# avianphysics/avian

Measured on NVIDIA H100. Metric: physics steps/sec on 100k-cube stack (broad phase + solver stage per step), higher is better.
Workload: dtype f32

## Files before the change

avian_b200/csrc/solver_dev.cuh:

```cuda
#pragma once
#include <cuda_pipeline.h>

#include "../../include/avian_b200.h"
#include "avn_math.cuh"

namespace avn {

enum { CP_N = 0, CP_T1 = 1, CP_TV = 2, CP_IDX = 3, CP_PT0 = 4, CP_PLANES = CP_PT0 + 3 * AVN_MAX_MANIFOLD_POINTS };
#define CP_ROW(k, r) (CP_PT0 + 3 * (k) + (r))
enum { CI_NP_MASK = 0x7, CI_ZERO1 = 1 << 4, CI_ZERO2 = 1 << 5, CI_NONDYN = 1 << 6, CI_TANGENT = 1 << 7,
       CI_VER1 = 1 << 8, CI_VER2 = 1 << 9 };
enum { BF_LOCK_MASK = 0x3f, BF_HAS_SOLVER_BODY = 1 << 8, BF_KINEMATIC = 1 << 9, BF_GYRO = 1 << 10, BF_DYNAMIC = 1 << 11,
       BF_CUSTOM_VEL = 1 << 12, BF_CUSTOM_POS = 1 << 13, BF_DOMINANCE_SHIFT = 16 };

enum { JP_IDX = 0,
       JP_R1 = 1,
       JP_R2 = 2,
       JP_CD = 3,
       JP_RD = 4,
       JP_A1 = 5,
       JP_A2 = 6,
       JP_B1 = 7,
       JP_B2 = 8,
       JP_LP = 9,
// ... 245 lines not shown
        case WV_WARM: return base + 1u + r;
        case WV_SOLVE: return base + 1u + unsigned(1 + it) * k + r;
        case WV_IP: return base + 1u + unsigned(1 + iters) * k;
        default: return base + 2u + unsigned(1 + iters) * k + r;
    }
}
__device__ __forceinline__ unsigned ld_acquire(const unsigned* p) {
    unsigned v;
    asm volatile("ld.acquire.gpu.global.u32 %0, [%1];" : "=r"(v) : "l"(p) : "memory");
    return v;
}
__device__ __forceinline__ void st_relaxed(unsigned* p, unsigned v) { asm volatile("st.relaxed.gpu.global.u32 [%0], %1;" ::"l"(p), "r"(v) : "memory"); }
__device__ __forceinline__ void fence_acq_rel() { asm volatile("fence.acq_rel.gpu;" ::: "memory"); }
__device__ __forceinline__ Vec4<float> ld4_cg(const Vec4<float>* p) {
    float4 v = __ldcg(reinterpret_cast<const float4*>(p));
    return mk4<float>(v.x, v.y, v.z, v.w);
}
__device__ __forceinline__ Vec4<double> ld4_cg(const Vec4<double>* p) {
    double2 a = __ldcg(reinterpret_cast<const double2*>(p)), b = __ldcg(reinterpret_cast<const double2*>(p) + 1);
    return mk4<double>(a.x, a.y, b.x, b.y);
}
template <bool WAVE, class S> __device__ __forceinline__ Vec4<S> ldm(const Vec4<S>* p) { return WAVE ? ld4_cg(p) : ld4(p); }
template <bool WAVE, class S> __device__ __forceinline__ Vec4<S> pc_load(const Vec4<S>* p) { return ldm<WAVE>(p); }

template <bool EXACT = true>
__device__ __forceinline__ void wave_wait(const unsigned* ver, bool need1, int b1, unsigned e1, bool need2, int b2, unsigned e2, int* watchdog,
                                          unsigned* seen1 = nullptr, unsigned* seen2 = nullptr) {
    for (unsigned spins = 0;; ++spins) {
        if (need1) { const unsigned v = ld_acquire(ver + b1); need1 = EXACT ? v != e1 : v < e1; if (seen1) *seen1 = v; }
        if (need2) { const unsigned v = ld_acquire(ver + b2); need2 = EXACT ? v != e2 : v < e2; if (seen2) *seen2 = v; }
        if (__all_sync(0xffffffffu, !(need1 || need2))) break;
        if (spins > (1u << 22)) { *watchdog = 1; break; }
    }
}
__device__ __forceinline__ void wave_publish(unsigned* ver, bool need1, int b1, unsigned e1, bool need2, int b2, unsigned e2) {
    fence_acq_rel();
    if (need1) st_relaxed(ver + b1, e1 + 1u);
    if (need2) st_relaxed(ver + b2, e2 + 1u);
}

constexpr int STAGE_ROWS = 3 * AVN_MAX_MANIFOLD_POINTS;
template <class S> __device__ __forceinline__ Vec4<S>* stage_base() {
    extern __shared__ __align__(32) unsigned char avn_stage_raw[];
    return reinterpret_cast<Vec4<S>*>(avn_stage_raw);
}
__device__ __forceinline__ void stage_copy(Vec4<float>* dst, const Vec4<float>* src) { __pipeline_memcpy_async(dst, src, 16); }
__device__ __forceinline__ void stage_copy(Vec4<double>* dst, const Vec4<double>* src) {
    __pipeline_memcpy_async(dst, src, 16);
    __pipeline_memcpy_async(reinterpret_cast<char*>(dst) + 16, reinterpret_cast<const char*>(src) + 16, 16);
}
template <class S> __host__ __device__ constexpr size_t stage_bytes(int threads, int max_points = AVN_MAX_MANIFOLD_POINTS) {
    return size_t(4 * max_points) * threads * sizeof(Vec4<S>);
}

template <class S, int PASS, int MAXP = AVN_MAX_MANIFOLD_POINTS>
__device__ __forceinline__ void contact_item(const DevSolver<S>& d, int slot) {
    const size_t MP = size_t(d.Mpad);
    Vec4<S>* c = d.cst + slot;
    Vec4<S> hidx = ld4(&c[CP_IDX * MP]);
    const int info = as_int(hidx.z);
    const int np = info & CI_NP_MASK;
    if (np == 0) return;
    const int b1 = as_int(hidx.x), b2 = as_int(hidx.y);
    Vec4<S> hn = mk4<S>(0, 0, 0, 0), ht1 = hn, htv = hn;
    BodyInertia<S> in1 = zero_inertia<S>(), in2 = zero_inertia<S>();
    Vec4<S> PC[MAXP];
    constexpr bool SOLVE = (PASS == PASS_SOLVE_BIAS || PASS == PASS_RELAX);
    Vec4<S>* const stage = stage_base<S>() + threadIdx.x;
    const int T = blockDim.x;
#define ROW_A(k) stage[(3 * (k) + 0) * T]
#define ROW_B(k) stage[(3 * (k) + 1) * T]
#define ROW_D(k) stage[(3 * (k) + 2) * T]
    {
        hn = ld4(&c[CP_N * MP]);
        ht1 = ld4(&c[CP_T1 * MP]);
        if (SOLVE) htv = ld4(&c[CP_TV * MP]);
        if (!(info & CI_ZERO1)) in1 = unpack_inertia(ld4(&d.inr[2 * b1]), ld4(&d.inr[2 * b1 + 1]));
        if (!(info & CI_ZERO2)) in2 = unpack_inertia(ld4(&d.inr[2 * b2]), ld4(&d.inr[2 * b2 + 1]));
#pragma unroll
        for (int k = 0; k < MAXP; ++k) {
            if (k < np) {
                stage_copy(&ROW_A(k), &c[size_t(CP_ROW(k, 0)) * MP]);
                stage_copy(&ROW_B(k), &c[size_t(CP_ROW(k, 1)) * MP]);
                if (PASS == PASS_RESTITUTION || (SOLVE && (info & CI_TANGENT))) stage_copy(&ROW_D(k), &c[size_t(CP_ROW(k, 2)) * MP]);
            }
        }
    }
    __pipeline_commit();
    Vec4<S> l1 = ld4(&d.vel[2 * b1]), a1 = ld4(&d.vel[2 * b1 + 1]);
    Vec4<S> l2 = ld4(&d.vel[2 * b2]), a2 = ld4(&d.vel[2 * b2 + 1]);
    Vec4<S> dp1, dq1, dp2, dq2;
    if (SOLVE) {
        dp1 = ld4(&d.dlt[2 * b1]); dq1 = ld4(&d.dlt[2 * b1 + 1]);
        dp2 = ld4(&d.dlt[2 * b2]); dq2 = ld4(&d.dlt[2 * b2 + 1]);
    }
#pragma unroll
    for (int k = 0; k < MAXP; ++k)
        if (k < np) PC[k] = pc_load<false>(pc_ptr(d, k, slot));
    __pipeline_wait_prior(0);
    V3<S> v1 = xyz(l1), w1 = xyz(a1), v2 = xyz(l2), w2 = xyz(a2);
    const V3<S> n = xyz(hn), t1 = xyz(ht1);
    const V3<S> t2 = cross(t1, n);

    if (PASS == PASS_WARM) {
#pragma unroll
        for (int k = 0; k < MAXP; ++k) {
// ... 63 lines not shown
                            nx = limit * (nx / l);
                            ny = limit * (ny / l);
                        }
                        S dx = nx - PC[k].z, dy = ny - PC[k].w;
                        PC[k].z = nx;
                        PC[k].w = ny;
                        imp = dx * t1 + dy * t2;
                    }
                    apply_impulse(v1, w1, v2, w2, in1, in2, r1, r2, imp);
                }
            }
        }
    } else {
        const S e = ht1.w;
        if (e == S(0)) return;
        const int iterations = np > 1 ? d.rest_iters : 1;
        for (int it = 0; it < iterations; ++it) {
#pragma unroll
            for (int k = 0; k < MAXP; ++k) {
                if (k < np) {
                    const Vec4<S> PAk = ROW_A(k), PBk = ROW_B(k), PDk = ROW_D(k);
                    if (PDk.w > -d.rest_threshold || PC[k].y == S(0)) continue;
                    V3<S> r1 = xyz(PAk), r2 = xyz(PBk);
                    V3<S> relv = (v2 + cross(w2, r2)) - (v1 + cross(w1, r1));
                    S vn = dot(relv, n);
                    S impulse = -PBk.w * (vn + e * PDk.w);
                    S new_impulse = avn_max(PC[k].x + impulse, S(0));
                    impulse = new_impulse - PC[k].x;
                    PC[k].x = new_impulse;
                    PC[k].y = PC[k].y + impulse;
                    apply_impulse(v1, w1, v2, w2, in1, in2, r1, r2, impulse * n);
                }
            }
        }
    }
    if (PASS != PASS_WARM) {
#pragma unroll
        for (int k = 0; k < MAXP; ++k)
            if (k < np) pc_store(pc_ptr(d, k, slot), PC[k]);
    }
    if (!(info & CI_ZERO1)) {
        st4(&d.vel[2 * b1], mk4<S>(v1.x, v1.y, v1.z, S(0)));
        st4(&d.vel[2 * b1 + 1], mk4<S>(w1.x, w1.y, w1.z, S(0)));
    }
    if (!(info & CI_ZERO2)) {
        st4(&d.vel[2 * b2], mk4<S>(v2.x, v2.y, v2.z, S(0)));
        st4(&d.vel[2 * b2 + 1], mk4<S>(w2.x, w2.y, w2.z, S(0)));
    }
#undef ROW_A
#undef ROW_B
#undef ROW_D
}

template <class S, int PASS, int MAXP>
__device__ __forceinline__ void wave_contact_item(const DevSolver<S>& d, int slot, int s, int it, bool relax) {
    constexpr bool SOLVE = PASS == PASS_SOLVE_BIAS;
    relax = SOLVE && relax;
    const size_t MP = size_t(d.Mpad);
    const Vec4<S>* c = d.cst + slot;
    const Vec4<S> hidx = ld4(&c[CP_IDX * MP]);
    const int info = as_int(hidx.z);
    const int np = info & CI_NP_MASK;
    const int b1 = as_int(hidx.x), b2 = as_int(hidx.y);
    Vec4<S>* const stage = stage_base<S>() + threadIdx.x;
    const int T = blockDim.x;
#define ROW_A(k) stage[(3 * (k) + 0) * T]
#define ROW_B(k) stage[(3 * (k) + 1) * T]
#define ROW_D(k) stage[(3 * (k) + 2) * T]
#define ROW_PC(k) stage[(3 * MAXP + (k)) * T]
    Vec4<S> hn = mk4<S>(0, 0, 0, 0), ht1 = hn, htv = hn;
    BodyInertia<S> in1 = zero_inertia<S>(), in2 = zero_inertia<S>();
    if (np != 0) {
        hn = ld4(&c[CP_N * MP]);
        ht1 = ld4(&c[CP_T1 * MP]);
        if (SOLVE) htv = ld4(&c[CP_TV * MP]);
        if (!(info & CI_ZERO1)) in1 = unpack_inertia(ld4(&d.inr[2 * b1]), ld4(&d.inr[2 * b1 + 1]));
        if (!(info & CI_ZERO2)) in2 = unpack_inertia(ld4(&d.inr[2 * b2]), ld4(&d.inr[2 * b2 + 1]));
#pragma unroll 1
        for (int k = 0; k < np; ++k) {
            stage_copy(&ROW_A(k), &c[size_t(CP_ROW(k, 0)) * MP]);
            stage_copy(&ROW_B(k), &c[size_t(CP_ROW(k, 1)) * MP]);
            if (SOLVE && (info & CI_TANGENT)) stage_copy(&ROW_D(k), &c[size_t(CP_ROW(k, 2)) * MP]);
        }
    }
    __pipeline_commit();
    const bool ver1 = np != 0 && (info & CI_VER1), ver2 = np != 0 && (info & CI_VER2);
    const int rk = as_int(hidx.w);
    const int k1 = (rk >> 8) & 0xff, k2 = (rk >> 24) & 0xff;
    const int kind = SOLVE ? (relax ? WV_RELAX : WV_SOLVE) : WV_WARM;
    const unsigned e1 = wave_event(kind, it, s, d.iters, k1, rk & 0xff);
    const unsigned e2 = wave_event(kind, it, s, d.iters, k2, (rk >> 16) & 0xff);
    int* const watchdog = d.any_restitution + FLAG_WAVE;
    const V3<S> n = xyz(hn), t1 = xyz(ht1);
    const Soft<S> soft = (info & CI_NONDYN) ? d.soft_nondyn : d.soft_dyn;
    unsigned biased_points = 0;
    unsigned seen1 = 0u, seen2 = 0u;

    if (SOLVE) {
        AVN_TRACE_T(t_d0);
        const int sd = relax ? s : s - 1;
        if (sd >= 0)
            wave_wait<false>(d.ver, ver1, b1, wave_event(WV_IP, 0, sd, d.iters, k1, 0) + 1u, ver2, b2, wave_event(WV_IP, 0, sd, d.iters, k2, 0) + 1u,
                             watchdog, &seen1, &seen2);
        __pipeline_wait_prior(0);
        if (np != 0) {
            const Vec4<S> dp1 = ld4_cg(&d.dlt[2 * b1]), dq1 = ld4_cg(&d.dlt[2 * b1 + 1]);
            const Vec4<S> dp2 = ld4_cg(&d.dlt[2 * b2]), dq2 = ld4_cg(&d.dlt[2 * b2 + 1]);
            Q4<S> q1; q1.x = dq1.x; q1.y = dq1.y; q1.z = dq1.z; q1.w = dq1.w;
            Q4<S> q2; q2.x = dq2.x; q2.y = dq2.y; q2.z = dq2.z; q2.w = dq2.w;
            const V3<S> delta_translation = xyz(dp2) - xyz(dp1);
#pragma unroll
            for (int k = 0; k < MAXP; ++k) {
                if (k >= np) break;
                const Vec4<S> PAk = ROW_A(k), PBk = ROW_B(k);
                V3<S> rr1 = qrot(q1, xyz(PAk)), rr2 = qrot(q2, xyz(PBk));
                V3<S> dsep = delta_translation + (rr2 - rr1);
                const S separation = dot(dsep, n) + PAk.w;
                const S meff = PBk.w;
                const bool separated = separation > S(0), biased = !separated && !relax;
                ROW_A(k).w = separated ? separation / d.h : biased ? avn_max(soft.bias * separation, -d.max_overlap_speed) : S(-0.0);
                ROW_B(k).w = biased ? soft.mass_scale * meff : meff;
                biased_points |= unsigned(biased) << k;
            }
        }
#ifdef AVN_WAVE_TRACE
        if (np != 0 && ROW_A(0).w == S(1.2345e33)) d.any_restitution[1] = 2;
        AVN_TRACE_ADD(d, 5, clock64() - t_d0);
#endif
    }

    AVN_TRACE_T(t_w0);
    wave_wait(d.ver, ver1 && seen1 != e1, b1, e1, ver2 && seen2 != e2, b2, e2, watchdog);
    AVN_TRACE_ADD(d, 0, clock64() - t_w0);
    if (np == 0) return;
    AVN_TRACE_T(t_l0);
    const Vec4<S> l1 = ld4_cg(&d.vel[2 * b1]), a1 = ld4_cg(&d.vel[2 * b1 + 1]);
    const Vec4<S> l2 = ld4_cg(&d.vel[2 * b2]), a2 = ld4_cg(&d.vel[2 * b2 + 1]);
    {
        Vec4<S> pc[MAXP];
#pragma unroll
        for (int k = 0; k < MAXP; ++k)
            if (k < np) pc[k] = pc_load<true>(pc_ptr(d, k, slot));
#pragma unroll
        for (int k = 0; k < MAXP; ++k)
            if (k < np) ROW_PC(k) = pc[k];
    }
    if (!SOLVE) __pipeline_wait_prior(0);
#ifdef AVN_WAVE_TRACE
    if ((l1.x + a1.x + l2.x + a2.x) == S(1.2345e33)) d.any_restitution[1] = 2;
    AVN_TRACE_T(t_c0);
    AVN_TRACE_ADD(d, 1, t_c0 - t_l0);
#endif
    V3<S> v1 = xyz(l1), w1 = xyz(a1), v2 = xyz(l2), w2 = xyz(a2);
    const V3<S> t2 = cross(t1, n);

    if (!SOLVE) {
#pragma unroll 1
        for (int k = 0; k < np; ++k) {
            const Vec4<S> PAk = ROW_A(k), PBk = ROW_B(k), pck = ROW_PC(k);
            V3<S> r1 = xyz(PAk), r2 = xyz(PBk);
            S tx = (info & CI_TANGENT) ? pck.z : S(0), ty = (info & CI_TANGENT) ? pck.w : S(0);
            V3<S> p = d.warm_coeff * ((pck.x * n + tx * t1) + ty * t2);
            apply_impulse(v1, w1, v2, w2, in1, in2, r1, r2, p);
        }
    } else {
        const bool tangent = (info & CI_TANGENT) != 0;
#pragma unroll 1
        for (int k = 0; k < np; ++k) {
            const Vec4<S> PAk = ROW_A(k), PBk = ROW_B(k);
            Vec4<S> pck = ROW_PC(k);
            V3<S> r1 = xyz(PAk), r2 = xyz(PBk);
            V3<S> relv = (v2 + cross(w2, r2)) - (v1 + cross(w1, r1));
            S vn = dot(relv, n);
            S acc = pck.x;
            const S C = ((biased_points >> k) & 1u) ? soft.impulse_scale * acc : S(0);
            S impulse = -PBk.w * (vn + PAk.w) - C;
            S new_impulse = avn_max(acc + impulse, S(0));
            impulse = new_impulse - acc;
            pck.x = new_impulse;
            pck.y = pck.y + new_impulse;
            if (tangent) ROW_PC(k) = pck;
            else pc_store(pc_ptr(d, k, slot), pck);
            apply_impulse(v1, w1, v2, w2, in1, in2, r1, r2, impulse * n);
        }
        if (tangent) {
            const S friction = hn.w;
            const V3<S> surf = xyz(htv);
#pragma unroll 1
            for (int k = 0; k < np; ++k) {
                const Vec4<S> PAk = ROW_A(k), PBk = ROW_B(k), PDk = ROW_D(k);
                Vec4<S> pck = ROW_PC(k);
                V3<S> r1 = xyz(PAk), r2 = xyz(PBk);
                V3<S> relv = (v2 + cross(w2, r2)) - (v1 + cross(w1, r1));
                S limit = friction * pck.x;
                relv = relv + surf;
                S ts1 = dot(relv, t1), ts2 = dot(relv, t2);
                S t11 = ts1 * ts1, t22 = ts2 * ts2, t12 = ts1 * ts2;
                S inv = (t11 * PDk.x + t22 * PDk.y) + t12 * PDk.z;
                S em = (t11 + t22) * (S(1) / inv);
                V3<S> imp = zero3<S>();
                if (avn_finite(em)) {
                    S nx = pck.z - em * ts1, ny = pck.w - em * ts2;
                    S l2 = nx * nx + ny * ny;
                    if (l2 > limit * limit) {
                        S l = avn_sqrt(l2);
                        nx = limit * (nx / l);
                        ny = limit * (ny / l);
                    }
                    S dx = nx - pck.z, dy = ny - pck.w;
                    pck.z = nx;
                    pck.w = ny;
                    imp = dx * t1 + dy * t2;
                }
                pc_store(pc_ptr(d, k, slot), pck);
                apply_impulse(v1, w1, v2, w2, in1, in2, r1, r2, imp);
            }
        }
    }
#ifdef AVN_WAVE_TRACE
    if ((v1.x + v2.x + w1.x + w2.x) == S(1.2345e33)) d.any_restitution[1] = 2;
    AVN_TRACE_T(t_s0);
    AVN_TRACE_ADD(d, 2, t_s0 - t_c0);
#endif
    if (!(info & CI_ZERO1)) {
        st4(&d.vel[2 * b1], mk4<S>(v1.x, v1.y, v1.z, S(0)));
        st4(&d.vel[2 * b1 + 1], mk4<S>(w1.x, w1.y, w1.z, S(0)));
    }
    if (!(info & CI_ZERO2)) {
        st4(&d.vel[2 * b2], mk4<S>(v2.x, v2.y, v2.z, S(0)));
        st4(&d.vel[2 * b2 + 1], mk4<S>(w2.x, w2.y, w2.z, S(0)));
    }
    wave_publish(d.ver, ver1, b1, e1, ver2, b2, e2);
#ifdef AVN_WAVE_TRACE
    AVN_TRACE_ADD(d, 3, clock64() - t_s0);
    AVN_TRACE_ADD(d, 4, 1);
#endif
#undef ROW_A
#undef ROW_B
#undef ROW_D
#undef ROW_PC
}

template <class S, bool WAVE = false>
__device__ __forceinline__ void integrate_velocity_item(const DevSolver<S>& d, int i, int s = 0) {
    const bool in_range = i < d.B;
    int f = 0;
    if (in_range) f = as_int(ld4(&d.inr[2 * i]).y);
    const bool live = in_range && (f & BF_HAS_SOLVER_BODY);
    const bool integrate = live && !(f & BF_CUSTOM_VEL) && !(f & BF_KINEMATIC), gyro = integrate && (f & BF_GYRO);
    Vec4<S> li = mk4<S>(0, 0, 0, 0), ai = li;
    Q4<S> rot0; rot0.x = rot0.y = rot0.z = rot0.w = S(0);
    Sym3<S> il; il.m00 = il.m01 = il.m02 = il.m11 = il.m12 = il.m22 = S(0);
    if (integrate) { li = ld4(&d.itg[2 * i]); ai = ld4(&d.itg[2 * i + 1]); }
    if (gyro) {
        rot0 = ldq(d.rotation, i);
        il.m00 = d.inv_inertia_local[6 * i]; il.m01 = d.inv_inertia_local[6 * i + 1]; il.m02 = d.inv_inertia_local[6 * i + 2];
        il.m11 = d.inv_inertia_local[6 * i + 3]; il.m12 = d.inv_inertia_local[6 * i + 4]; il.m22 = d.inv_inertia_local[6 * i + 5];
    }
    const S max_lin = live && d.max_lin ? d.max_lin[i] : S(0), max_ang = live && d.max_ang ? d.max_ang[i] : S(0);
    const int bnd = live && d.bnd_of ? d.bnd_of[i] : -1;
    unsigned e = 0;
    if (WAVE) {
        if (live) e = wave_event(WV_IV, 0, s, d.iters, d.deg[i], 0);
        wave_wait(d.ver, live, i, e, false, 0, 0u, d.any_restitution + 1);
    }
    if (!live) return;
    Vec4<S> l = ldm<WAVE>(&d.vel[2 * i]), a = ldm<WAVE>(&d.vel[2 * i + 1]);
    V3<S> v = xyz(l), w = xyz(a);
    bool touched = false;
    if (integrate) {
        v = v * li.w;
        w = w * ai.w;
        v = v + xyz(li);
        w = w + xyz(ai);
        if (gyro) {
            Vec4<S> dq4 = ldm<WAVE>(&d.dlt[2 * i + 1]);
            Q4<S> dq; dq.x = dq4.x; dq.y = dq4.y; dq.z = dq4.z; dq.w = dq4.w;
            Q4<S> rot = qmul(dq, rot0);
            V3<S> lw = qrot(qconj(rot), w);
            Sym3<S> tensor = sym_inverse_or_zero(il);
            V3<S> L = smul(tensor, lw);
            V3<S> Ln = L - d.h * cross(lw, L);
            S l2 = len2(Ln);
            if (l2 == S(0)) {
                w = zero3<S>();
            } else {
                Ln = Ln * avn_sqrt(len2(L) / l2);
                w = qrot(rot, smul(il, Ln));
            }
        }
        touched = true;
    }
// ... 131 lines not shown
```

avian_b200/csrc/solver_host.cu:

```cuda
#include <algorithm>
#include <cmath>
#include <cstdlib>
#include <cstring>

#include "context.hpp"
#include "joint_schedule.hpp"
#include "solver_kernels.cuh"

namespace avn {

namespace {

template <class S>
Soft<S> softness(S damping_ratio, S hz, S delta_secs) {
    S double_damping_ratio = S(2) * damping_ratio;
    S angular_frequency = S(6.283185307179586476925286766559) * hz;
    S a1 = double_damping_ratio + angular_frequency * delta_secs;
    S a2 = angular_frequency * delta_secs * a1;
    S a3 = S(1) / (S(1) + a2);
    Soft<S> s;
    s.bias = angular_frequency / a1;
    s.mass_scale = a2 * a3;
    s.impulse_scale = a3;
    return s;
// ... 120 lines not shown
        UPS(b_ad_, bc.angular_damping, B, S, ang_damp);
        UPS(b_gs_, bc.gravity_scale, B, S, grav_scale);
        UPB(b_la_, bc.linear_acceleration, 3 * B, S, lin_acc);
        UPB(b_aa_, bc.angular_acceleration, 3 * B, S, ang_acc);
        UPS(b_ml_, bc.max_linear_speed, B, S, max_lin);
        UPS(b_ma_, bc.max_angular_speed, B, S, max_ang);
#undef UPS
#undef UPB
        bcols_.kind = d.kind; bcols_.locked = d.locked; bcols_.dominance = d.dominance; bcols_.integ_flags = d.integ_flags;
        bcols_.position = d.position; bcols_.rotation = d.rotation; bcols_.linvel = d.linvel; bcols_.angvel = d.angvel; bcols_.inv_mass = d.inv_mass;
        bcols_.inv_inertia_local = d.inv_inertia_local; bcols_.com = d.com; bcols_.lin_damp = d.lin_damp; bcols_.ang_damp = d.ang_damp;
        bcols_.grav_scale = d.grav_scale; bcols_.lin_acc = d.lin_acc; bcols_.ang_acc = d.ang_acc; bcols_.max_lin = d.max_lin; bcols_.max_ang = d.max_ang;
        bcols_.count = B;
        return AVN_OK;
    }
    AvnStatus build_joint_schedule(const AvnBodyColumns& bc, const AvnJointSet& js);
    AvnStatus launch_range(uint32_t first, uint32_t count, uint32_t flags);
    bool ccd_active() const { return ccd_ && ccd_->active(); }
    CcdBase* ccd_ = nullptr;
    ContactsBase* ccd_contacts_ = nullptr;
    bool from_store_ = false;
    double length_unit_ = 1;
    template <int OP> void launch_phase(int begin, int count, bool serial = false) {
        if (count <= 0) return;
        int grid = serial ? 1 : std::min((count + kBlock - 1) / kBlock, sm_count_ * 8);
        const bool contact_op = OP == OP_WARM || OP == OP_SOLVE_BIAS || OP == OP_RELAX || OP == OP_RESTITUTION;
        const size_t smem = contact_op ? stage_bytes<S>(kBlock) : 0;
        if (smem > 48 * 1024) cudaFuncSetAttribute(phase_kernel<S, OP>, cudaFuncAttributeMaxDynamicSharedMemorySize, int(smem));
        phase_kernel<S, OP><<<grid, kBlock, smem, stream_>>>(dev_, begin, count, serial ? 1 : 0);
        ++launches_;
    }
    template <int OP> void launch_contact_pass() {
        const int* off = dev_.color_off;
        launch_phase<OP>(off[AVN_COLOR_OVERFLOW], dev_.color_len[AVN_COLOR_OVERFLOW], true);
        for (int c = 0; c < AVN_COLOR_OVERFLOW; ++c) launch_phase<OP>(off[c], dev_.color_len[c]);
    }

    cudaStream_t stream_;
    ErrorSink* err_;
    uint32_t cfg_flags_;
    int sm_count_ = 132;
    bool coop_ok_ = false, use_mega_ = true, use_wave_ = true, l2_persist_ = false;
    size_t l2_persist_bytes_ = 0, l2_window_max_ = 0;
    int mega_grid_ = 0, mega_bps_ = 3, mega_maxp_ = 0, mega_sel_bps_ = 0;
    bool force_wave_ = false;

    template <int MAXP> const void* mega_variant(int bps) const {
        switch (bps) {
            case 2: return (const void*)step_megakernel<S, 2, MAXP>;
            case 4: return (const void*)step_megakernel<S, 4, MAXP>;
            default: return (const void*)step_megakernel<S, 3, MAXP>;
        }
    }
    static size_t mega_smem_bytes(int maxp) { return stage_bytes<S>(MEGA_BLOCK, maxp); }
    bool select_megakernel(int max_points, int bps = 0) {
        const int maxp = max_points <= 1 ? 1 : AVN_MAX_MANIFOLD_POINTS;
        if (bps == 0) bps = mega_bps_;
        if (maxp == mega_maxp_ && bps == mega_sel_bps_) return mega_grid_ > 0;
        mega_maxp_ = maxp;
        mega_sel_bps_ = bps;
        mega_fn_ = maxp == 1 ? mega_variant<1>(bps) : mega_variant<AVN_MAX_MANIFOLD_POINTS>(bps);
        const size_t smem = mega_smem_bytes(maxp);
        int per_sm = 0;
        mega_grid_ = 0;
        if (cudaFuncSetAttribute(mega_fn_, cudaFuncAttributeMaxDynamicSharedMemorySize, int(smem)) == cudaSuccess &&
            cudaOccupancyMaxActiveBlocksPerMultiprocessor(&per_sm, mega_fn_, MEGA_BLOCK, smem) == cudaSuccess && per_sm > 0)
            mega_grid_ = per_sm * sm_count_;
        else
            (void)cudaGetLastError();
        if (getenv("AVN_DEBUG_GRID")) fprintf(stderr, "[avn] megakernel bps=%d maxp=%d: %d blocks/SM resident, grid %d, %zu B dynamic smem\n", bps, maxp, per_sm, mega_grid_, smem);
        return mega_grid_ > 0;
    }
    int max_np_ = AVN_MAX_MANIFOLD_POINTS;
    const void* mega_fn_ = nullptr;
    cudaEvent_t ev_[EV_COUNT];
    AvnTimings tm_{};
    uint32_t launches_ = 0, exchanges_ = 0;
    size_t h2d_bytes_ = 0;
    bool uploaded_ = false, ran_ = false, host_any_restitution_ = false, prepared_ = false, mega_step_ = false;
    DevBuf bnd_of_, bnd_body_, bnd_slot_, bnd_owner_, vel_ref_, bnd_table_, bnd_gathered_, bnd_agree_;
    int* h_agree_ = nullptr;
    int agreed_rest_ = 0;
    bool agreed_valid_ = false;
    int bnd_n_ = 0, bnd_rank_ = 0, bnd_world_ = 1, step_bps_ = 0;
    size_t bnd_slots_ = 0;

    DevSolver<S> dev_{};
    AvnBodyColumns hb_{};
    struct ManifoldSource {
        size_t M = 0, P = 0;
        const uint32_t* color_offsets = nullptr;
        const int32_t* body1 = nullptr; const int32_t* body2 = nullptr;
        const void* friction = nullptr; const void* restitution = nullptr; const void* tangent_velocity = nullptr; const void* normal = nullptr;
        const uint32_t* point_offsets = nullptr;
        const uint32_t* edge = nullptr; const uint8_t* edge_point_count = nullptr;
        const void* anchor1 = nullptr; const void* anchor2 = nullptr; const void* penetration = nullptr; const void* normal_speed = nullptr;
        void* ws_normal = nullptr; void* ws_tangent = nullptr; void* normal_impulse = nullptr;
        bool resident = false;
        bool list_restitution = false;
        void* out_ws_normal = nullptr; void* out_ws_tangent = nullptr; void* out_normal_impulse = nullptr;
    };
    AvnStatus upload_impl(const AvnStepParams* prm, AvnBodyColumns* bc, const ManifoldSource* src, AvnJointSet* js);
    ManifoldSource hm_{};
    DevBuf m_pbegin_, m_pend_;
    AvnJointSet hj_{};
    bool have_m_ = false, have_j_ = false;

// ... 613 lines not shown
        if ((st = comm->all_reduce_max_i32(bnd_agree_.as<int>(), 1)) != AVN_OK) return st;
        AVN_CUDA(cudaMemcpyAsync(h_agree_, bnd_agree_.p, sizeof(int), cudaMemcpyDeviceToHost, stream_));
        AVN_CUDA(cudaStreamSynchronize(stream_));
        any_rest = *h_agree_;
        agreed_rest_ = any_rest;
        agreed_valid_ = true;
    }
    const uint32_t substeps = uint32_t(dev_.substeps);
    for (uint32_t s = 0; s < substeps; ++s) {
        if ((st = run_range(s, 1, s == 0 ? AVN_RUN_PREPARE : 0u)) != AVN_OK) return st;
        if ((st = exchange()) != AVN_OK) return st;
    }
    if (substeps == 0 && (st = run_range(0, 0, AVN_RUN_PREPARE)) != AVN_OK) return st;
    if (any_rest) {
        if ((st = boundary_snapshot()) != AVN_OK) return st;
        if ((st = run_range(substeps, 0, AVN_RUN_RESTITUTION)) != AVN_OK) return st;
        if ((st = exchange()) != AVN_OK) return st;
    }
    return run_range(substeps, 0, AVN_RUN_FINALIZE);
}

template <class S>
AvnStatus Solver<S>::download() {
    if (!ran_) return err_->fail(AVN_ERR_INVALID_ARGUMENT, "avn_solver_download before avn_solver_run");
    const size_t B = hb_.count;
    cudaEventRecord(ev_[EV_D2H0], stream_);
    if (B) {
        AVN_CUDA(cudaMemcpyAsync(hb_.position, dev_.out_position, 3 * B * sizeof(S), cudaMemcpyDeviceToHost, stream_));
        AVN_CUDA(cudaMemcpyAsync(hb_.rotation, dev_.out_rotation, 4 * B * sizeof(S), cudaMemcpyDeviceToHost, stream_));
        AVN_CUDA(cudaMemcpyAsync(hb_.linear_velocity, dev_.out_linvel, 3 * B * sizeof(S), cudaMemcpyDeviceToHost, stream_));
        AVN_CUDA(cudaMemcpyAsync(hb_.angular_velocity, dev_.out_angvel, 3 * B * sizeof(S), cudaMemcpyDeviceToHost, stream_));
    }
    if (have_m_ && !hm_.resident) {
        const size_t P = hm_.P;
        AVN_CUDA(cudaMemcpyAsync(hm_.ws_normal, dev_.p_out_ws_normal, P * sizeof(S), cudaMemcpyDeviceToHost, stream_));
        AVN_CUDA(cudaMemcpyAsync(hm_.ws_tangent, dev_.p_out_ws_tangent, 2 * P * sizeof(S), cudaMemcpyDeviceToHost, stream_));
        AVN_CUDA(cudaMemcpyAsync(hm_.normal_impulse, dev_.p_normal_impulse, P * sizeof(S), cudaMemcpyDeviceToHost, stream_));
    }
    if (have_j_) {
        for (int t = 0; t < AVN_JOINT_TYPE_COUNT; ++t) {
            const size_t n = hj_.types[t].count;
            if (n && dev_.jforce[t]) AVN_CUDA(cudaMemcpyAsync(hj_.types[t].force, dev_.jforce[t], 3 * n * sizeof(S), cudaMemcpyDeviceToHost, stream_));
            if (n && dev_.jtorque[t]) AVN_CUDA(cudaMemcpyAsync(hj_.types[t].torque, dev_.jtorque[t], 3 * n * sizeof(S), cudaMemcpyDeviceToHost, stream_));
        }
    }
    int flags_host[2] = {0, 0};
    AVN_CUDA(cudaMemcpyAsync(flags_host, dev_.any_restitution, sizeof flags_host, cudaMemcpyDeviceToHost, stream_));
    cudaEventRecord(ev_[EV_D2H1], stream_);
    AVN_CUDA(cudaStreamSynchronize(stream_));
#ifdef AVN_WAVE_TRACE
    {
        unsigned long long tr[8];
        cudaMemcpy(tr, dev_.any_restitution + FLAG_WORDS, sizeof tr, cudaMemcpyDeviceToHost);
        if (tr[4]) fprintf(stderr, "[avn wave trace] contact item-warps %llu  avg cycles: stage 1 (wait deltas + separations + coefficients) %.0f  wait %.0f  loads %.0f  compute %.0f  "
                           "store+publish %.0f\n", tr[4], double(tr[5]) / tr[4], double(tr[0]) / tr[4], double(tr[1]) / tr[4], double(tr[2]) / tr[4], double(tr[3]) / tr[4]);
    }
#endif
    if (flags_host[1] == WAVE_BAD_COLOURING)
        return err_->fail(AVN_ERR_INVALID_ARGUMENT, "manifolds: invalid colouring — a body with a SolverBody appears twice in one graph colour (or carries more than 254 "
                                                    "constraints): the colours are not conflict-free, the results of this step are not reliable");
    if (flags_host[1] == WAVE_WATCHDOG) return err_->fail(AVN_ERR_CUDA, "wavefront scheduler watchdog fired: results are invalid (set AVN_LAUNCH_MODE=barrier)");
    float ms = 0;
    if (cudaEventElapsedTime(&ms, ev_[EV_H2D0], ev_[EV_H2D1]) == cudaSuccess) tm_.h2d_ms = ms;
    if (cudaEventElapsedTime(&ms, ev_[EV_RUN0], ev_[EV_PREP]) == cudaSuccess) tm_.prepare_ms = ms;
    if (cudaEventElapsedTime(&ms, ev_[EV_PREP], ev_[EV_LOOP]) == cudaSuccess) tm_.substep_loop_ms = ms;
    if (cudaEventElapsedTime(&ms, ev_[EV_LOOP], ev_[EV_RUN1]) == cudaSuccess) tm_.finalize_ms = ms;
    if (cudaEventElapsedTime(&ms, ev_[EV_D2H0], ev_[EV_D2H1]) == cudaSuccess) tm_.d2h_ms = ms;
    if (cudaEventElapsedTime(&ms, ev_[EV_RUN0], ev_[EV_RUN1]) == cudaSuccess) tm_.total_ms = ms;
    tm_.kernel_launches = launches_;
    tm_.contact_constraint_count = uint32_t(dev_.M);
    tm_.joint_levels = uint32_t(dev_.n_levels);
    uint32_t ac = 0;
    for (int c = 0; c < AVN_GRAPH_COLOR_COUNT; ++c) ac += dev_.color_len[c] > 0;
    tm_.active_colors = ac;
    tm_.launch_mode = !mega_step_ ? AVN_LAUNCH_PHASES : (dev_.wave ? AVN_LAUNCH_MEGA_WAVE : AVN_LAUNCH_MEGA_BARRIER);
    return AVN_OK;
}

}

SolverBase* make_solver(uint32_t scalar_bits, cudaStream_t stream, ErrorSink* err, uint32_t cfg_flags, int device) {
    if (scalar_bits == 32) return new Solver<float>(stream, err, cfg_flags, device);
    if (scalar_bits == 64) return new Solver<double>(stream, err, cfg_flags, device);
    return nullptr;
}

}
```

avian_b200/csrc/solver_kernels.cuh:

```cuda
#pragma once
#include <cooperative_groups.h>

#include "joints_dev.cuh"

namespace avn {
namespace cg = cooperative_groups;

constexpr int MEGA_BLOCK = 128;

enum PhaseOp {
    OP_PREPARE_BODY = 0, OP_PREPARE_CONSTRAINT, OP_PREPARE_JOINT, OP_INTEGRATE_VEL, OP_INTEGRATE_POS, OP_WARM, OP_SOLVE_BIAS,
    OP_RELAX, OP_RESTITUTION, OP_SOLVE_JOINT, OP_PROJECT_VEL, OP_DAMP_JOINT, OP_WRITEBACK_BODY, OP_STORE_IMPULSE, OP_JOINT_FORCE,
    OP_WAVE_RANK, OP_WAVE_PACK
};

template <class S, int OP, int MAXP = AVN_MAX_MANIFOLD_POINTS>
__device__ __forceinline__ void run_item(const DevSolver<S>& d, int i) {
    if (OP == OP_PREPARE_BODY) prepare_body_item(d, i);
    else if (OP == OP_PREPARE_CONSTRAINT) prepare_constraint_item(d, i);
    else if (OP == OP_PREPARE_JOINT) prepare_joint_item(d, i);
    else if (OP == OP_INTEGRATE_VEL) integrate_velocity_item(d, i);
    else if (OP == OP_INTEGRATE_POS) { integrate_position_item(d, i); if (d.J > 0) store_pre_solve_item(d, i); }
    else if (OP == OP_WARM) contact_item<S, PASS_WARM, MAXP>(d, i);
    else if (OP == OP_SOLVE_BIAS) contact_item<S, PASS_SOLVE_BIAS, MAXP>(d, i);
    else if (OP == OP_RELAX) contact_item<S, PASS_RELAX, MAXP>(d, i);
    else if (OP == OP_RESTITUTION) contact_item<S, PASS_RESTITUTION, MAXP>(d, i);
    else if (OP == OP_SOLVE_JOINT) solve_joint_item(d, i);
    else if (OP == OP_PROJECT_VEL) {
        project_velocity_item(d, i);
        if (i == 0)
            for (int k = 0; k < 2 * AVN_JOINT_TYPE_COUNT; ++k) d.jdummy[k] = Vec4<S>{};
    }
    else if (OP == OP_DAMP_JOINT) damp_joint_item(d, d.jdamp_slot[i]);
    else if (OP == OP_WRITEBACK_BODY) writeback_body_item(d, i);
    else if (OP == OP_STORE_IMPULSE) store_impulse_item(d, i);
    else if (OP == OP_JOINT_FORCE) joint_force_item(d, i);
    else if (OP == OP_WAVE_RANK) wave_rank_item(d, i);
    else if (OP == OP_WAVE_PACK) wave_pack_item(d, i);
}

template <class S, int OP>
__global__ void __launch_bounds__(256) phase_kernel(const __grid_constant__ DevSolver<S> d, int begin, int count, int serial) {
    if (serial) {
        if (blockIdx.x == 0 && threadIdx.x == 0)
            for (int i = 0; i < count; ++i) run_item<S, OP>(d, begin + i);
        return;
    }
    for (int i = blockIdx.x * blockDim.x + threadIdx.x; i < count; i += gridDim.x * blockDim.x) run_item<S, OP>(d, begin + i);
}

template <class S, int OP, int MAXP = AVN_MAX_MANIFOLD_POINTS>
__device__ __noinline__ void grid_phase(const DevSolver<S>& d, int begin, int count) {
    for (int i = blockIdx.x * blockDim.x + threadIdx.x; i < count; i += gridDim.x * blockDim.x) run_item<S, OP, MAXP>(d, begin + i);
}

template <class S, int OP, int MAXP = AVN_MAX_MANIFOLD_POINTS>
__device__ __noinline__ void grid_serial(const DevSolver<S>& d, int begin, int count) {
    for (int i = 0; i < count; ++i) run_item<S, OP, MAXP>(d, begin + i);
}

template <class S, int OP, int MAXP = AVN_MAX_MANIFOLD_POINTS>
__device__ __forceinline__ void grid_contact_pass(const DevSolver<S>& d, cg::grid_group& grid) {
    const int ov = d.color_off[AVN_COLOR_OVERFLOW], ovn = d.color_len[AVN_COLOR_OVERFLOW];
    if (ovn > 0) {
        if (blockIdx.x == 0 && threadIdx.x == 0) grid_serial<S, OP, MAXP>(d, ov, ovn);
        grid.sync();
    }
    for (int c = 0; c < AVN_COLOR_OVERFLOW; ++c) {
        const int b = d.color_off[c], n = d.color_len[c];
        if (n <= 0) continue;
        grid_phase<S, OP, MAXP>(d, b, n);
        grid.sync();
    }
}

constexpr int WAVE_CHUNK = 32;
template <class S, int PASS, int MAXP, int BPS>
__device__ __noinline__ void wave_contact_chunk(const DevSolver<S>& d, int slot, int s, int it, bool relax) {
    wave_contact_item<S, PASS, MAXP>(d, slot, s, it, relax);
}
template <class S, int BPS, int MAXP>
__device__ __noinline__ void wave_iv_chunk(const DevSolver<S>& d, int i, int s) { integrate_velocity_item<S, true>(d, i, s); }
template <class S, int BPS, int MAXP>
__device__ __noinline__ void wave_ip_chunk(const DevSolver<S>& d, int i, int s) { integrate_position_item<S, true>(d, i, s); }

template <class S, int MAXP, int BPS>
__device__ __forceinline__ void wave_substep_loop(const DevSolver<S>& d) {
    const int lane = threadIdx.x & 31;
    const long long warps = (long long)gridDim.x * (blockDim.x >> 5);
    const long long warp_id = (long long)blockIdx.x * (blockDim.x >> 5) + (threadIdx.x >> 5);
    const int body_chunks = (d.B + WAVE_CHUNK - 1) / WAVE_CHUNK, slot_chunks = d.Mpad / WAVE_CHUNK;
    const int first_chunks = body_chunks;
    const int front_passes = 1 + d.iters;
    const long long per_substep = (long long)first_chunks + body_chunks + (long long)(front_passes + 1) * slot_chunks;
    const long long total = per_substep * d.sub_end;
    for (long long g = per_substep * d.sub_begin + warp_id; g < total; g += warps) {
        const int s = int(g / per_substep);
        long long r = g - (long long)s * per_substep;
        if (r < first_chunks) {
            wave_iv_chunk<S, BPS, MAXP>(d, int(r) * WAVE_CHUNK + lane, s);
            continue;
        }
        r -= first_chunks;
        if (r < (long long)front_passes * slot_chunks) {
            const int pass = int(r / slot_chunks), slot = int(r - (long long)pass * slot_chunks) * WAVE_CHUNK + lane;
            if (pass == 0) wave_contact_chunk<S, PASS_WARM, MAXP, BPS>(d, slot, s, 0, false);
            else wave_contact_chunk<S, PASS_SOLVE_BIAS, MAXP, BPS>(d, slot, s, pass - 1, false);
            continue;
        }
        r -= (long long)front_passes * slot_chunks;
        if (r < body_chunks) { wave_ip_chunk<S, BPS, MAXP>(d, int(r) * WAVE_CHUNK + lane, s); continue; }
        r -= body_chunks;
        wave_contact_chunk<S, PASS_SOLVE_BIAS, MAXP, BPS>(d, int(r) * WAVE_CHUNK + lane, s, 0, true);
    }
}

template <class S, int BPS, int MAXP>
__global__ void __launch_bounds__(MEGA_BLOCK, BPS) step_megakernel(const __grid_constant__ DevSolver<S> d) {
    cg::grid_group grid = cg::this_grid();
    if (d.do_prepare) {
        grid_phase<S, OP_PREPARE_BODY>(d, 0, d.B + 1);
        grid.sync();
        grid_phase<S, OP_PREPARE_CONSTRAINT>(d, 0, d.M);
        grid_phase<S, OP_PREPARE_JOINT>(d, 0, d.J);
        grid.sync();
        if (d.wave) {
            for (int c = 0; c < AVN_COLOR_OVERFLOW; ++c) {
                if (d.color_len[c] <= 0) continue;
                grid_phase<S, OP_WAVE_RANK>(d, d.color_off[c], d.color_len[c]);
                grid.sync();
            }
            grid_phase<S, OP_WAVE_PACK>(d, 0, d.Mpad);
            grid.sync();
        }
    }
    const bool wave = d.wave && *reinterpret_cast<volatile int*>(d.any_restitution + 1) == 0;
    if (wave && d.sub_end > d.sub_begin) {
        wave_substep_loop<S, MAXP, BPS>(d);
        grid.sync();
    }
    for (int sub = d.sub_begin; sub < (wave ? 0 : d.sub_end); ++sub) {
        grid_phase<S, OP_INTEGRATE_VEL>(d, 0, d.B);
        grid.sync();
        if (d.M > 0) {
            grid_contact_pass<S, OP_WARM, MAXP>(d, grid);
            for (int it = 0; it < d.iters; ++it) grid_contact_pass<S, OP_SOLVE_BIAS, MAXP>(d, grid);
        }
        grid_phase<S, OP_INTEGRATE_POS>(d, 0, d.B);
        grid.sync();
        if (d.M > 0) grid_contact_pass<S, OP_RELAX, MAXP>(d, grid);
        if (d.J > 0) {
            for (int l = 0; l < d.n_levels; ++l) {
                const int b = d.level_off[l], n = d.level_off[l + 1] - b;
                grid_phase<S, OP_SOLVE_JOINT>(d, b, n);
                grid.sync();
            }
            grid_phase<S, OP_PROJECT_VEL>(d, 0, d.B);
            grid.sync();
            for (int l = 0; l < d.n_damp_levels; ++l) {
                const int b = d.damp_level_off[l], n = d.damp_level_off[l + 1] - b;
                grid_phase<S, OP_DAMP_JOINT>(d, b, n);
                grid.sync();
            }
        }
    }
    if (d.do_restitution && d.M > 0 && *d.any_restitution) grid_contact_pass<S, OP_RESTITUTION, MAXP>(d, grid);
// ... 9 lines not shown
```

Before: 441.7.

## Prefetch next wave chunk's contact header and rows into double-buffered shared memory

```diff
diff --git a/avian_b200/csrc/solver_dev.cuh b/avian_b200/csrc/solver_dev.cuh
--- a/avian_b200/csrc/solver_dev.cuh
+++ b/avian_b200/csrc/solver_dev.cuh
@@ -321,6 +321,12 @@
 template <class S> __host__ __device__ constexpr size_t stage_bytes(int threads, int max_points = AVN_MAX_MANIFOLD_POINTS) {
     return size_t(4 * max_points) * threads * sizeof(Vec4<S>);
 }
+enum { WT_HDR = 0, WT_ROWS = 1 };
+template <class S> __host__ __device__ constexpr int wave_bufs() { return sizeof(S) == 4 ? 2 : 1; }
+__host__ __device__ constexpr int wave_buf_rows(int max_points) { return 3 * max_points + 1; }
+template <class S> __host__ __device__ constexpr size_t wave_tile_bytes(int threads, int max_points) {
+    return size_t(WT_ROWS + wave_bufs<S>() * wave_buf_rows(max_points) + max_points) * threads * sizeof(Vec4<S>);
+}
 
 template <class S, int PASS, int MAXP = AVN_MAX_MANIFOLD_POINTS>
 __device__ __forceinline__ void contact_item(const DevSolver<S>& d, int slot) {
@@ -490,37 +496,55 @@
 #undef ROW_D
 }
 
+
+template <int N> __device__ __forceinline__ void wave_rows_wait() {
+    __pipeline_wait_prior(N);
+    asm volatile("" ::: "memory");
+}
+template <class S, int MAXP>
+__device__ __forceinline__ void wave_stage_rows(Vec4<S>* rows, int T, const Vec4<S>* c, size_t MP, int np, bool rows_d) {
+    stage_copy(&rows[3 * MAXP * T], &c[CP_N * MP]);
+#pragma unroll 1
+    for (int k = 0; k < np; ++k) {
+        stage_copy(&rows[(3 * k + 0) * T], &c[size_t(CP_ROW(k, 0)) * MP]);
+        stage_copy(&rows[(3 * k + 1) * T], &c[size_t(CP_ROW(k, 1)) * MP]);
+        if (rows_d) stage_copy(&rows[(3 * k + 2) * T], &c[size_t(CP_ROW(k, 2)) * MP]);
+    }
+}
+
 template <class S, int PASS, int MAXP>
-__device__ __forceinline__ void wave_contact_item(const DevSolver<S>& d, int slot, int s, int it, bool relax) {
+__device__ __forceinline__ void wave_contact_item(const DevSolver<S>& d, int slot, int s, int it, bool relax, int buf, bool pre, int nslot,
+                                                  bool nsolve) {
     constexpr bool SOLVE = PASS == PASS_SOLVE_BIAS;
+    constexpr int NB = wave_bufs<S>(), BUF = wave_buf_rows(MAXP);
     relax = SOLVE && relax;
+    AVN_TRACE_T(t_h0);
     const size_t MP = size_t(d.Mpad);
     const Vec4<S>* c = d.cst + slot;
-    const Vec4<S> hidx = ld4(&c[CP_IDX * MP]);
+    Vec4<S>* const col = stage_base<S>() + threadIdx.x;
+    const int T = blockDim.x;
+    Vec4<S>* const rows = col + (WT_ROWS + (NB == 2 ? buf : 0) * BUF) * T;
+    const bool staged = NB == 2 && pre;
+    const Vec4<S> hidx = pre ? col[WT_HDR * T] : ld4(&c[CP_IDX * MP]);
     const int info = as_int(hidx.z);
     const int np = info & CI_NP_MASK;
     const int b1 = as_int(hidx.x), b2 = as_int(hidx.y);
-    Vec4<S>* const stage = stage_base<S>() + threadIdx.x;
-    const int T = blockDim.x;
-#define ROW_A(k) stage[(3 * (k) + 0) * T]
-#define ROW_B(k) stage[(3 * (k) + 1) * T]
-#define ROW_D(k) stage[(3 * (k) + 2) * T]
-#define ROW_PC(k) stage[(3 * MAXP + (k)) * T]
-    Vec4<S> hn = mk4<S>(0, 0, 0, 0), ht1 = hn, htv = hn;
+#define ROW_A(k) rows[(3 * (k) + 0) * T]
+#define ROW_B(k) rows[(3 * (k) + 1) * T]
+#define ROW_D(k) rows[(3 * (k) + 2) * T]
+#define ROW_N rows[3 * MAXP * T]
+#define ROW_PC(k) col[(WT_ROWS + NB * BUF + (k)) * T]
+    Vec4<S> ht1 = mk4<S>(0, 0, 0, 0), htv = ht1;
     BodyInertia<S> in1 = zero_inertia<S>(), in2 = zero_inertia<S>();
     if (np != 0) {
-        hn = ld4(&c[CP_N * MP]);
         ht1 = ld4(&c[CP_T1 * MP]);
         if (SOLVE) htv = ld4(&c[CP_TV * MP]);
         if (!(info & CI_ZERO1)) in1 = unpack_inertia(ld4(&d.inr[2 * b1]), ld4(&d.inr[2 * b1 + 1]));
         if (!(info & CI_ZERO2)) in2 = unpack_inertia(ld4(&d.inr[2 * b2]), ld4(&d.inr[2 * b2 + 1]));
-#pragma unroll 1
-        for (int k = 0; k < np; ++k) {
-            stage_copy(&ROW_A(k), &c[size_t(CP_ROW(k, 0)) * MP]);
-            stage_copy(&ROW_B(k), &c[size_t(CP_ROW(k, 1)) * MP]);
-            if (SOLVE && (info & CI_TANGENT)) stage_copy(&ROW_D(k), &c[size_t(CP_ROW(k, 2)) * MP]);
-        }
-    }
+        if (!staged) wave_stage_rows<S, MAXP>(rows, T, c, MP, np, SOLVE && (info & CI_TANGENT));
+    }
+    if (!staged) __pipeline_commit();
+    if (nslot >= 0) stage_copy(&col[WT_HDR * T], &d.cst[CP_IDX * MP + nslot]);
     __pipeline_commit();
     const bool ver1 = np != 0 && (info & CI_VER1), ver2 = np != 0 && (info & CI_VER2);
     const int rk = as_int(hidx.w);
@@ -529,10 +553,14 @@
     const unsigned e1 = wave_event(kind, it, s, d.iters, k1, rk & 0xff);
     const unsigned e2 = wave_event(kind, it, s, d.iters, k2, (rk >> 16) & 0xff);
     int* const watchdog = d.any_restitution + FLAG_WAVE;
-    const V3<S> n = xyz(hn), t1 = xyz(ht1);
     const Soft<S> soft = (info & CI_NONDYN) ? d.soft_nondyn : d.soft_dyn;
     unsigned biased_points = 0;
     unsigned seen1 = 0u, seen2 = 0u;
+    Vec4<S> hn;
+#ifdef AVN_WAVE_TRACE
+    if ((ht1.x + in1.inv_mass.x + in2.inv_mass.x) == S(1.2345e33)) d.any_restitution[1] = 2;
+    AVN_TRACE_ADD(d, 6, clock64() - t_h0);
+#endif
 
     if (SOLVE) {
         AVN_TRACE_T(t_d0);
@@ -540,8 +568,10 @@
         if (sd >= 0)
             wave_wait<false>(d.ver, ver1, b1, wave_event(WV_IP, 0, sd, d.iters, k1, 0) + 1u, ver2, b2, wave_event(WV_IP, 0, sd, d.iters, k2, 0) + 1u,
                              watchdog, &seen1, &seen2);
-        __pipeline_wait_prior(0);
+        wave_rows_wait<1>();
+        hn = ROW_N;
         if (np != 0) {
+            const V3<S> n = xyz(hn);
             const Vec4<S> dp1 = ld4_cg(&d.dlt[2 * b1]), dq1 = ld4_cg(&d.dlt[2 * b1 + 1]);
             const Vec4<S> dp2 = ld4_cg(&d.dlt[2 * b2]), dq2 = ld4_cg(&d.dlt[2 * b2 + 1]);
             Q4<S> q1; q1.x = dq1.x; q1.y = dq1.y; q1.z = dq1.z; q1.w = dq1.w;
@@ -570,6 +600,18 @@
     AVN_TRACE_T(t_w0);
     wave_wait(d.ver, ver1 && seen1 != e1, b1, e1, ver2 && seen2 != e2, b2, e2, watchdog);
     AVN_TRACE_ADD(d, 0, clock64() - t_w0);
+    if (nslot >= 0) {
+        AVN_TRACE_T(t_a0);
+        wave_rows_wait<0>();
+        if (NB == 2) {
+            const Vec4<S> nh = col[WT_HDR * T];
+            const int ninfo = as_int(nh.z), nnp = ninfo & CI_NP_MASK;
+            if (nnp != 0)
+                wave_stage_rows<S, MAXP>(col + (WT_ROWS + (buf ^ 1) * BUF) * T, T, d.cst + nslot, MP, nnp, nsolve && (ninfo & CI_TANGENT));
+            __pipeline_commit();
+        }
+        AVN_TRACE_ADD(d, 7, clock64() - t_a0);
+    }
     if (np == 0) return;
     AVN_TRACE_T(t_l0);
     const Vec4<S> l1 = ld4_cg(&d.vel[2 * b1]), a1 = ld4_cg(&d.vel[2 * b1 + 1]);
@@ -583,13 +625,17 @@
         for (int k = 0; k < MAXP; ++k)
             if (k < np) ROW_PC(k) = pc[k];
     }
-    if (!SOLVE) __pipeline_wait_prior(0);
+    if (!SOLVE) {
+        if (nslot < 0) wave_rows_wait<0>();
+        hn = ROW_N;
+    }
 #ifdef AVN_WAVE_TRACE
     if ((l1.x + a1.x + l2.x + a2.x) == S(1.2345e33)) d.any_restitution[1] = 2;
     AVN_TRACE_T(t_c0);
     AVN_TRACE_ADD(d, 1, t_c0 - t_l0);
 #endif
     V3<S> v1 = xyz(l1), w1 = xyz(a1), v2 = xyz(l2), w2 = xyz(a2);
+    const V3<S> n = xyz(hn), t1 = xyz(ht1);
     const V3<S> t2 = cross(t1, n);
 
     if (!SOLVE) {
@@ -676,6 +722,7 @@
 #undef ROW_A
 #undef ROW_B
 #undef ROW_D
+#undef ROW_N
 #undef ROW_PC
 }
 
diff --git a/avian_b200/csrc/solver_host.cu b/avian_b200/csrc/solver_host.cu
--- a/avian_b200/csrc/solver_host.cu
+++ b/avian_b200/csrc/solver_host.cu
@@ -196,7 +196,7 @@
             default: return (const void*)step_megakernel<S, 3, MAXP>;
         }
     }
-    static size_t mega_smem_bytes(int maxp) { return stage_bytes<S>(MEGA_BLOCK, maxp); }
+    static size_t mega_smem_bytes(int maxp) { return wave_tile_bytes<S>(MEGA_BLOCK, maxp); }
     bool select_megakernel(int max_points, int bps = 0) {
         const int maxp = max_points <= 1 ? 1 : AVN_MAX_MANIFOLD_POINTS;
         if (bps == 0) bps = mega_bps_;
@@ -916,8 +916,9 @@
     {
         unsigned long long tr[8];
         cudaMemcpy(tr, dev_.any_restitution + FLAG_WORDS, sizeof tr, cudaMemcpyDeviceToHost);
-        if (tr[4]) fprintf(stderr, "[avn wave trace] contact item-warps %llu  avg cycles: stage 1 (wait deltas + separations + coefficients) %.0f  wait %.0f  loads %.0f  compute %.0f  "
-                           "store+publish %.0f\n", tr[4], double(tr[5]) / tr[4], double(tr[0]) / tr[4], double(tr[1]) / tr[4], double(tr[2]) / tr[4], double(tr[3]) / tr[4]);
+        if (tr[4]) fprintf(stderr, "[avn wave trace] contact item-warps %llu  avg cycles: header %.0f  stage 1 (wait deltas + separations + coefficients) %.0f  "
+                           "next chunk %.0f  wait %.0f  loads %.0f  compute %.0f  store+publish %.0f\n", tr[4], double(tr[6]) / tr[4], double(tr[5]) / tr[4],
+                           double(tr[7]) / tr[4], double(tr[0]) / tr[4], double(tr[1]) / tr[4], double(tr[2]) / tr[4], double(tr[3]) / tr[4]);
     }
 #endif
     if (flags_host[1] == WAVE_BAD_COLOURING)
diff --git a/avian_b200/csrc/solver_kernels.cuh b/avian_b200/csrc/solver_kernels.cuh
--- a/avian_b200/csrc/solver_kernels.cuh
+++ b/avian_b200/csrc/solver_kernels.cuh
@@ -76,13 +76,36 @@
 
 constexpr int WAVE_CHUNK = 32;
 template <class S, int PASS, int MAXP, int BPS>
-__device__ __noinline__ void wave_contact_chunk(const DevSolver<S>& d, int slot, int s, int it, bool relax) {
-    wave_contact_item<S, PASS, MAXP>(d, slot, s, it, relax);
+__device__ __noinline__ void wave_contact_chunk(const DevSolver<S>& d, int slot, int s, int it, bool relax, int buf, bool pre, int nslot,
+                                                bool nsolve) {
+    wave_contact_item<S, PASS, MAXP>(d, slot, s, it, relax, buf, pre, nslot, nsolve);
 }
 template <class S, int BPS, int MAXP>
 __device__ __noinline__ void wave_iv_chunk(const DevSolver<S>& d, int i, int s) { integrate_velocity_item<S, true>(d, i, s); }
 template <class S, int BPS, int MAXP>
 __device__ __noinline__ void wave_ip_chunk(const DevSolver<S>& d, int i, int s) { integrate_position_item<S, true>(d, i, s); }
+
+struct WaveChunk { int kind, s, first, it; };
+__device__ __forceinline__ WaveChunk wave_chunk(long long g, long long per_substep, int body_chunks, int slot_chunks, int front_passes) {
+    WaveChunk c;
+    c.s = int(g / per_substep);
+    c.it = 0;
+    long long r = g - (long long)c.s * per_substep;
+    if (r < body_chunks) { c.kind = WV_IV; c.first = int(r) * WAVE_CHUNK; return c; }
+    r -= body_chunks;
+    if (r < (long long)front_passes * slot_chunks) {
+        const int pass = int(r / slot_chunks);
+        c.kind = pass == 0 ? WV_WARM : WV_SOLVE;
+        c.it = pass == 0 ? 0 : pass - 1;
+        c.first = int(r - (long long)pass * slot_chunks) * WAVE_CHUNK;
+        return c;
+    }
+    r -= (long long)front_passes * slot_chunks;
+    if (r < body_chunks) { c.kind = WV_IP; c.first = int(r) * WAVE_CHUNK; return c; }
+    c.kind = WV_RELAX;
+    c.first = int(r - body_chunks) * WAVE_CHUNK;
+    return c;
+}
 
 template <class S, int MAXP, int BPS>
 __device__ __forceinline__ void wave_substep_loop(const DevSolver<S>& d) {
@@ -90,28 +113,26 @@
     const long long warps = (long long)gridDim.x * (blockDim.x >> 5);
     const long long warp_id = (long long)blockIdx.x * (blockDim.x >> 5) + (threadIdx.x >> 5);
     const int body_chunks = (d.B + WAVE_CHUNK - 1) / WAVE_CHUNK, slot_chunks = d.Mpad / WAVE_CHUNK;
-    const int first_chunks = body_chunks;
     const int front_passes = 1 + d.iters;
-    const long long per_substep = (long long)first_chunks + body_chunks + (long long)(front_passes + 1) * slot_chunks;
+    const long long per_substep = 2LL * body_chunks + (long long)(front_passes + 1) * slot_chunks;
     const long long total = per_substep * d.sub_end;
+    int buf = 0;
+    bool pre = false;
     for (long long g = per_substep * d.sub_begin + warp_id; g < total; g += warps) {
-        const int s = int(g / per_substep);
-        long long r = g - (long long)s * per_substep;
-        if (r < first_chunks) {
-            wave_iv_chunk<S, BPS, MAXP>(d, int(r) * WAVE_CHUNK + lane, s);
+        const WaveChunk c = wave_chunk(g, per_substep, body_chunks, slot_chunks, front_passes);
+        if (c.kind == WV_IV || c.kind == WV_IP) {
+            if (c.kind == WV_IV) wave_iv_chunk<S, BPS, MAXP>(d, c.first + lane, c.s);
+            else wave_ip_chunk<S, BPS, MAXP>(d, c.first + lane, c.s);
+            pre = false;
             continue;
         }
-        r -= first_chunks;
-        if (r < (long long)front_passes * slot_chunks) {
-            const int pass = int(r / slot_chunks), slot = int(r - (long long)pass * slot_chunks) * WAVE_CHUNK + lane;
-            if (pass == 0) wave_contact_chunk<S, PASS_WARM, MAXP, BPS>(d, slot, s, 0, false);
-            else wave_contact_chunk<S, PASS_SOLVE_BIAS, MAXP, BPS>(d, slot, s, pass - 1, false);
-            continue;
-        }
-        r -= (long long)front_passes * slot_chunks;
-        if (r < body_chunks) { wave_ip_chunk<S, BPS, MAXP>(d, int(r) * WAVE_CHUNK + lane, s); continue; }
-        r -= body_chunks;
-        wave_contact_chunk<S, PASS_SOLVE_BIAS, MAXP, BPS>(d, int(r) * WAVE_CHUNK + lane, s, 0, true);
+        WaveChunk n{WV_IV, 0, 0, 0};
+        if (g + warps < total) n = wave_chunk(g + warps, per_substep, body_chunks, slot_chunks, front_passes);
+        const int nslot = (n.kind == WV_IV || n.kind == WV_IP) ? -1 : n.first + lane;
+        if (c.kind == WV_WARM) wave_contact_chunk<S, PASS_WARM, MAXP, BPS>(d, c.first + lane, c.s, 0, false, buf, pre, nslot, n.kind != WV_WARM);
+        else wave_contact_chunk<S, PASS_SOLVE_BIAS, MAXP, BPS>(d, c.first + lane, c.s, c.it, c.kind == WV_RELAX, buf, pre, nslot, n.kind != WV_WARM);
+        pre = nslot >= 0;
+        buf ^= 1;
     }
 }
 
```

Result: slower. 428.7 (median of 6 runs) (-2.9%).
